# Mateng0228/Leak-det-gnn

Hardware: AMD Instinct MI355X
Metric: windowed graphs/sec fwd+bwd on L-TOWN-A (higher is better)
Workload: dtype fp32; 1 GPU; L-TOWN-A detector training step (BASELINE configs[2]); graph=L-TOWN-A, nodes=661, edge_columns=1532, pipes=764, windows_per_rank=256, global_batch=256, feat=64, gnn_layers=2, parallelism=dp1, launch=hipgraph (one replay per step, dropout re-drawn on device)

## Files before the change

include/leakgnn.h:

```cpp
#ifndef LEAKGNN_H
#define LEAKGNN_H

#include <stdint.h>

#ifdef __cplusplus
extern "C" {
#endif

typedef void* lg_stream_t;

enum {
    LG_OK = 0,
    LG_EINVAL = -1,
    LG_EUNSUPPORTED = -2,
    LG_EHIP = -3
};

#define LG_F_BIAS      0x01
#define LG_F_RELU      0x02
#define LG_F_DROPOUT   0x04
#define LG_F_MASK_IN   0x08
#define LG_F_MASK_OUT  0x10
#define LG_F_DX_SENSOR_ROWS 0x10000000
#define LG_F_NODE_MAJOR 0x20
#define LG_F_BF16 0x40
#define LG_SALT_SEED_PTR 0x80000000u
#define LG_F_F32_MFMA      0x00400000
#define LG_F_PC            0x00004000
#define LG_F_BF16X3        0x00008000
#define LG_F_NM3           0x00020000

int lg_abi_version(void);

int lg_reduce_batch_begin(void);
int lg_reduce_batch_flush(lg_stream_t stream);

int lg_stream_copy(const void* src, void* dst, int64_t bytes, lg_stream_t stream);

int lg_seed_slots_advance(uint64_t* slots, int64_t n, uint64_t* state, lg_stream_t stream);

int lg_graph_replay(void* graph_exec, int64_t n, lg_stream_t stream);
const char* lg_strerror(int code);

int lg_cross_entropy_fwd(const float* logits, const int64_t* target, int64_t B, int64_t C, int64_t ldx,
                         int64_t ignore_index, float* loss, float* lse, float* rowloss, unsigned* counter,
                         lg_stream_t stream);
int lg_cross_entropy_bwd(const float* logits, const int64_t* target, const float* lse, const float* grad_loss,
                         int64_t B, int64_t C, int64_t ldx, int64_t ignore_index, float* dlogits, int64_t ldd,
                         lg_stream_t stream);

int64_t lg_clip_adamw_workspace_bytes(const int64_t* sizes, int T);
int lg_clip_adamw(const int64_t* table, const int64_t* sizes, int T, float* step, float lr, float beta1,
                  float beta2, float eps, float weight_decay, float max_norm, float* norm_out, void* workspace, int64_t ws_bytes,
                  lg_stream_t stream);
int lg_clip_adamw_seeds(const int64_t* table, const int64_t* sizes, int T, float* step, float lr, float beta1,
                        float beta2, float eps, float weight_decay, float max_norm, float* norm_out, void* workspace,
                        int64_t ws_bytes, uint64_t* seed_slots, int64_t n_slots, uint64_t* seed_state,
                        lg_stream_t stream);

int lg_spin_errors(uint32_t* out, int reset);

int lg_timing_arm(int slot);
int lg_timing_disarm(void);
int lg_timing_elapsed(int slot, float* ms);

int64_t lg_graph_workspace_bytes(int64_t E, int64_t N);
int lg_graph_build(const int64_t* edge_index, int64_t E, int64_t N,
                   int add_self_loops, int normalize, float fill_value,
                   int32_t* rowptr, int32_t* col, float* w,
                   int32_t* rowptr_t, int32_t* col_t, float* w_t,
                   void* workspace, int64_t ws_bytes, lg_stream_t stream);

int64_t lg_graph_build_w_workspace_bytes(int64_t E, int64_t N);
int lg_graph_build_w(const int64_t* edge_index, const float* edge_weight, int64_t E, int64_t N,
                     int add_self_loops, int normalize, float fill_value,
                     int32_t* rowptr, int32_t* col, float* w, int32_t* eid,
                     int32_t* rowptr_t, int32_t* col_t, float* w_t, int32_t* eid_t, float* dis,
                     void* workspace, int64_t ws_bytes, lg_stream_t stream);
int lg_graph_reweight(const int32_t* rowptr, const int32_t* col, const int32_t* eid,
                      const int32_t* rowptr_t, const int32_t* col_t, const int32_t* eid_t,
                      const float* edge_weight, int64_t E, int64_t N, int normalize, float fill_value,
                      float* dis, float* w, float* w_t, lg_stream_t stream);
int64_t lg_gcn_norm_bwd_workspace_bytes(int64_t E, int64_t N);
int lg_gcn_norm_bwd(const float* G, const int32_t* rowptr, const int32_t* col, const int32_t* eid,
                    const int32_t* rowptr_t, const int32_t* col_t, const int32_t* eid_t,
                    const float* dis, const float* edge_weight, int64_t E, int64_t N, int normalize,
                    float fill_value, float* dedge_weight, void* workspace, int64_t ws_bytes,
                    lg_stream_t stream);

int lg_sddmm_cols(const int32_t* rowptr, const int32_t* col, const float* a, int64_t lda,
                  const float* b, int64_t ldb, float* out, int64_t N, int64_t C, lg_stream_t stream);

int lg_nm_table_build(const int32_t* rowptr, const int32_t* pairs, int64_t N, const int32_t* order,
                      int32_t* nodetab, lg_stream_t stream);

int lg_nm_table_sensor_mark(const int32_t* nodetab, const int32_t* pairs, int64_t N, int64_t nnz,
                            const int32_t* node_slot, int32_t* nodetab_out, int32_t* pairs_out, int32_t* pos_slot,
                            lg_stream_t stream);

int lg_rcm_order(const int64_t* edge_index, int64_t E, int64_t N, int32_t* order);

int64_t lg_incidence_workspace_bytes(int64_t P, int64_t N);
int lg_incidence_build(const int64_t* ends, int64_t P, int64_t N,
                       int32_t* inc_rowptr, int32_t* inc_item,
                       void* workspace, int64_t ws_bytes, lg_stream_t stream);

int lg_batchify_edge_index(const int64_t* edge_index, int64_t E, int64_t N, int64_t B,
                           int64_t* out, lg_stream_t stream);

int lg_node_init_fwd(const int32_t* sensor_slot, const float* proj, const float* bias, float* x0,
                     int64_t B, int64_t N, int64_t S, int64_t D,
                     int flags, float dropout_p, uint64_t seed, uint32_t salt, lg_stream_t stream);

int lg_node_init_proj_fwd(const int32_t* sensor_slot, const int64_t* sensor_idx, const float* h_s, const float* W,
                          const float* bias, float* x0, int64_t B, int64_t N, int64_t S, int64_t Ds, int64_t D,
                          int flags, float dropout_p, uint64_t seed, uint32_t salt, lg_stream_t stream);

int64_t lg_sensor_proj_bwd_workspace_bytes(int64_t B, int64_t S, int64_t Ds, int64_t D);
int lg_sensor_proj_bwd(const float* dx0, const int64_t* sensor_idx, const float* live, const float* h_s,
                       const float* W, const float* dbias_in, float* dh_s, float* dW, float* db, int64_t B,
                       int64_t N, int64_t S, int64_t Ds, int64_t D, int flags, void* workspace, int64_t ws_bytes,
                       lg_stream_t stream);

int64_t lg_linear_dw_workspace_bytes(int64_t K, int64_t M, int64_t N);
int lg_linear_dw(const float* dy, const float* x, int64_t K, int64_t M, int64_t N,
                 float* dw, float* db, void* workspace, int64_t ws_bytes, lg_stream_t stream);

int lg_gcn_fwd(const int32_t* rowptr, const int32_t* col, const float* w,
               const float* x, const float* W, const float* bias, float* y,
               int64_t B, int64_t N, int64_t D, int64_t nnz_cap,
               int flags, float dropout_p, uint64_t seed, uint32_t salt, lg_stream_t stream);

// ... 178 lines not shown
```

leak-det-gnn_amd/csrc/loss.hip:

```cpp
#include <algorithm>
#include "common.h"

namespace {

constexpr int kCeWaves = 4;
constexpr int kCeThreads = 64 * kCeWaves;
constexpr int kCePer = 16;
constexpr float kCeLseFine = 32.f;

__device__ __forceinline__ float wave_max(float v) {
#pragma unroll
    for (int o = 32; o > 0; o >>= 1) v = fmaxf(v, __shfl_xor(v, o));
    return v;
}
__device__ __forceinline__ float wave_sum(float v) {
#pragma unroll
    for (int o = 32; o > 0; o >>= 1) v += __shfl_xor(v, o);
    return v;
}

__device__ __forceinline__ void ce_mean_wave(float* rowloss, const int64_t* __restrict__ target, int64_t B,
                                             int64_t ignore, float* __restrict__ loss) {
    const int lane = threadIdx.x & 63;
    float acc = 0.f, cnt = 0.f;
    for (int64_t b0 = 0; b0 < B; b0 += 64) {
        const int64_t b = b0 + lane;
        float v = 0.f, c = 0.f;
        if (b < B) {
            v = __hip_atomic_load(rowloss + b, __ATOMIC_RELAXED, __HIP_MEMORY_SCOPE_AGENT);
            c = target[b] == ignore ? 0.f : 1.f;
        }
        acc += wave_sum(v);
        cnt += wave_sum(c);
    }
    if (lane == 0) loss[0] = acc / cnt;
}

__global__ void __launch_bounds__(kCeThreads)
k_ce_fwd(const float* __restrict__ x, const int64_t* __restrict__ target, int64_t B, int64_t C, int64_t ldx,
         int64_t ignore, float* __restrict__ lse, float* rowloss, unsigned* counter, float* __restrict__ loss) {
    __shared__ unsigned is_last;
    const int w = threadIdx.x >> 6, lane = threadIdx.x & 63;
    for (int64_t b = static_cast<int64_t>(blockIdx.x) * kCeWaves + w; b < B; b += static_cast<int64_t>(gridDim.x) * kCeWaves) {
        const float* row = x + b * ldx;
        float m = -__builtin_huge_valf(), s = 0.f;
        if (C <= 64 * kCePer) {
            float v[kCePer];
#pragma unroll
            for (int k = 0; k < kCePer; ++k) {
                const int64_t c = lane + 64 * k;
                v[k] = c < C ? row[c] : -__builtin_huge_valf();
            }
#pragma unroll
            for (int k = 0; k < kCePer; ++k) m = fmaxf(m, v[k]);
            m = wave_max(m);
#pragma unroll
            for (int k = 0; k < kCePer; ++k) s += lane + 64 * k < C ? expf(v[k] - m) : 0.f;
        } else {
            for (int64_t c = lane; c < C; c += 64) m = fmaxf(m, row[c]);
            m = wave_max(m);
            for (int64_t c = lane; c < C; c += 64) s += expf(row[c] - m);
        }
        s = wave_sum(s);
        const float ls = logf(s);
        const float l = m + ls;
        if (lane == 0) {
            const int64_t t = target[b];
            lse[b] = l;
            float rl = t == ignore ? 0.f : __builtin_nanf("");
            if (t >= 0 && t < C && t != ignore) rl = fabsf(l) < kCeLseFine ? l - row[t] : (m - row[t]) + ls;
            __hip_atomic_store(rowloss + b, rl, __ATOMIC_RELAXED, __HIP_MEMORY_SCOPE_AGENT);
        }
    }
    asm volatile("s_waitcnt vmcnt(0)" ::: "memory");
    __syncthreads();
    if (threadIdx.x == 0) {
        const unsigned old = __hip_atomic_fetch_add(counter, 1u, __ATOMIC_RELAXED, __HIP_MEMORY_SCOPE_AGENT);
        is_last = old + 1 == gridDim.x ? 1u : 0u;
    }
    __syncthreads();
    if (!is_last) return;
    if (w == 0) ce_mean_wave(rowloss, target, B, ignore, loss);
    if (threadIdx.x == 0) __hip_atomic_store(counter, 0u, __ATOMIC_RELAXED, __HIP_MEMORY_SCOPE_AGENT);
}

__global__ void __launch_bounds__(kCeThreads)
k_ce_bwd(const float* __restrict__ x, const int64_t* __restrict__ target, const float* __restrict__ lse,
         const float* __restrict__ gout, int64_t B, int64_t C, int64_t ldx, int64_t ignore, float* __restrict__ dx,
         int64_t ldd) {
    const int w = threadIdx.x >> 6, lane = threadIdx.x & 63;
    float cnt = 0.f;
    for (int64_t b0 = 0; b0 < B; b0 += 64) {
        const int64_t b = b0 + lane;
        cnt += wave_sum((b < B && target[b] != ignore) ? 1.f : 0.f);
    }
    const float g = gout[0] / cnt;
    for (int64_t b = static_cast<int64_t>(blockIdx.x) * kCeWaves + w; b < B; b += static_cast<int64_t>(gridDim.x) * kCeWaves) {
        const float* row = x + b * ldx;
        float* drow = dx + b * ldd;
        const int64_t t = target[b];
        const float l = lse[b];
        const float gi = t == ignore ? 0.f : g;
        const bool fine = fabsf(l) < kCeLseFine;
        if (C <= 64 * kCePer) {
            float v[kCePer];
#pragma unroll
            for (int k = 0; k < kCePer; ++k) {
                const int64_t c = lane + 64 * k;
                v[k] = c < C ? row[c] : 0.f;
            }
            if (fine) {
#pragma unroll
                for (int k = 0; k < kCePer; ++k) {
                    const int64_t c = lane + 64 * k;
                    if (c < C) drow[c] = gi * (expf(v[k] - l) - (c == t ? 1.f : 0.f));
                }
            } else {
                float m = -__builtin_huge_valf(), s = 0.f;
#pragma unroll
                for (int k = 0; k < kCePer; ++k) m = lane + 64 * k < C ? fmaxf(m, v[k]) : m;
                m = wave_max(m);
#pragma unroll
                for (int k = 0; k < kCePer; ++k) {
                    v[k] = lane + 64 * k < C ? expf(v[k] - m) : 0.f;
                    s += v[k];
                }
                const float rs = 1.f / wave_sum(s);
#pragma unroll
                for (int k = 0; k < kCePer; ++k) {
                    const int64_t c = lane + 64 * k;
                    if (c < C) drow[c] = gi * (v[k] * rs - (c == t ? 1.f : 0.f));
                }
            }
        } else if (fine) {
            for (int64_t c = lane; c < C; c += 64) drow[c] = gi * (expf(row[c] - l) - (c == t ? 1.f : 0.f));
        } else {
            float m = -__builtin_huge_valf(), s = 0.f;
            for (int64_t c = lane; c < C; c += 64) m = fmaxf(m, row[c]);
            m = wave_max(m);
            for (int64_t c = lane; c < C; c += 64) s += expf(row[c] - m);
            const float rs = 1.f / wave_sum(s);
            for (int64_t c = lane; c < C; c += 64) drow[c] = gi * (expf(row[c] - m) * rs - (c == t ? 1.f : 0.f));
        }
    }
}

}

extern "C" int lg_cross_entropy_fwd(const float* logits, const int64_t* target, int64_t B, int64_t C, int64_t ldx,
                                    int64_t ignore_index, float* loss, float* lse, float* rowloss, unsigned* counter,
                                    lg_stream_t stream) {
    if (B < 0 || C <= 0 || ldx < C || !loss || !counter) return LG_EINVAL;
    hipStream_t s = lg_stream(stream);
    if (B == 0) {
        return hipMemsetD32Async(reinterpret_cast<hipDeviceptr_t>(loss), 0x7FC00000, 1, s) == hipSuccess ? LG_OK
                                                                                                          : LG_EHIP;
    }
    if (!logits || !target || !lse || !rowloss) return LG_EINVAL;
    const int grid = static_cast<int>(std::min<int64_t>((B + kCeWaves - 1) / kCeWaves, lg_num_cus()));
    lg_launch(k_ce_fwd, grid, kCeThreads, 0, s, logits, target, B, C, ldx, ignore_index, lse, rowloss, counter, loss);
    LG_RET_IF_LAUNCH_FAILED();
    return LG_OK;
}

extern "C" int lg_cross_entropy_bwd(const float* logits, const int64_t* target, const float* lse,
                                    const float* grad_loss, int64_t B, int64_t C, int64_t ldx, int64_t ignore_index,
                                    float* dlogits, int64_t ldd, lg_stream_t stream) {
    if (B < 0 || C <= 0 || ldx < C || ldd < C || !grad_loss) return LG_EINVAL;
    if (B == 0) return LG_OK;
    if (!logits || !target || !lse || !dlogits) return LG_EINVAL;
    hipStream_t s = lg_stream(stream);
    const int grid = static_cast<int>(std::min<int64_t>((B + kCeWaves - 1) / kCeWaves, 4 * lg_num_cus()));
    lg_launch(k_ce_bwd, grid, kCeThreads, 0, s, logits, target, lse, grad_loss, B, C, ldx, ignore_index, dlogits, ldd);
    LG_RET_IF_LAUNCH_FAILED();
    return LG_OK;
}
```

leak-det-gnn_amd/csrc/optim.hip:

```cpp
#include <algorithm>
#include <cstdlib>
#include "common.h"

namespace {

constexpr int kOptThreads = 1024;
constexpr int kOptChunk = kOptThreads;
constexpr int kOptMaxTensors = 48;
constexpr uint32_t kOptPollLimit = 1u << 22;

struct AdamTensors {
    int64_t ptr[kOptMaxTensors][4];
    int64_t off[kOptMaxTensors + 1];
    int T;
};

__device__ __forceinline__ uint64_t opt_splitmix64(uint64_t z) {
    z += 0x9E3779B97F4A7C15ull;
    z = (z ^ (z >> 30)) * 0xBF58476D1CE4E5B9ull;
    z = (z ^ (z >> 27)) * 0x94D049BB133111EBull;
    return z ^ (z >> 31);
}
struct AdamSeeds {
    uint64_t* slots;
    uint64_t* state;
    int n;
};

enum : int {
    kAdamOne = 0,
    kAdamPartials = 1,
    kAdamNoNorm = 2,
};

__device__ __forceinline__ double opt_block_sum(double x, double* wsum) {
#pragma unroll
    for (int o = 32; o > 0; o >>= 1) x += __shfl_xor(x, o);
    if ((threadIdx.x & 63) == 0) wsum[threadIdx.x >> 6] = x;
    __syncthreads();
    double s = 0.0;
#pragma unroll
    for (int w = 0; w < kOptThreads / 64; ++w) s += wsum[w];
    __syncthreads();
    return s;
}

__device__ __forceinline__ int opt_tensor_of(const AdamTensors& a, int64_t e) {
    int t = 0;
    while (t < a.T && a.off[t + 1] <= e) ++t;
    return t;
}

__global__ void __launch_bounds__(kOptThreads) k_adam_partials(AdamTensors a, double* __restrict__ partials) {
    __shared__ double wsum[kOptThreads / 64];
    const int64_t e = static_cast<int64_t>(blockIdx.x) * kOptChunk + threadIdx.x;
    const int t = opt_tensor_of(a, e);
    double x = 0.0;
    if (t < a.T) x = reinterpret_cast<const float*>(a.ptr[t][1])[e - a.off[t]];
    const double s = opt_block_sum(x * x, wsum);
    if (threadIdx.x == 0) partials[blockIdx.x] = s;
}

template <int MODE>
__global__ void __launch_bounds__(kOptThreads)
k_adam(AdamTensors a, float* __restrict__ step, float lr, float beta1, float beta2, float eps, float wd,
       float max_norm, float* __restrict__ norm_out, double* __restrict__ partials, int skew, AdamSeeds seeds) {
    __shared__ uint32_t last;
    __shared__ double wsum[kOptThreads / 64];
    __shared__ float tsh;
    const int tid = threadIdx.x;
    const uint32_t G = gridDim.x;
    uint32_t* ctr = reinterpret_cast<uint32_t*>(step + 1);
    if (tid == 0) tsh = __hip_atomic_load(step, __ATOMIC_RELAXED, __HIP_MEMORY_SCOPE_AGENT) + 1.0f;
    if (MODE == kAdamNoNorm) __syncthreads();
    const int64_t e = static_cast<int64_t>(blockIdx.x) * kOptChunk + tid;
    const int t = opt_tensor_of(a, e);
    const bool live = t < a.T;
    const int64_t i = live ? e - a.off[t] : 0;
    float* p = live ? reinterpret_cast<float*>(a.ptr[t][0]) : nullptr;
    float* g = live ? reinterpret_cast<float*>(a.ptr[t][1]) : nullptr;
    float* m = live ? reinterpret_cast<float*>(a.ptr[t][2]) : nullptr;
    float* v = live ? reinterpret_cast<float*>(a.ptr[t][3]) : nullptr;
    if (MODE == kAdamOne && skew > 0 && (blockIdx.x & 1)) {
        for (int k = 0; k < skew; ++k) __builtin_amdgcn_s_sleep(127);
    }
    float gi = live ? g[i] : 0.0f;
    double norm = 0.0;
    if (MODE == kAdamOne) {
        const double s = opt_block_sum(static_cast<double>(gi) * gi, wsum);
        if (tid == 0) {
            partials[blockIdx.x] = s;
            __hip_atomic_fetch_add(ctr, 1u, __ATOMIC_RELEASE, __HIP_MEMORY_SCOPE_AGENT);
            uint32_t polls = 0;
            while (__hip_atomic_load(ctr, __ATOMIC_RELAXED, __HIP_MEMORY_SCOPE_AGENT) < G) {
                if (++polls > kOptPollLimit) {
                    __hip_atomic_fetch_or(reinterpret_cast<uint32_t*>(step + 2), 1u, __ATOMIC_RELAXED,
                                          __HIP_MEMORY_SCOPE_AGENT);
                    break;
                }
                __builtin_amdgcn_s_sleep(2);
            }
            __builtin_amdgcn_fence(__ATOMIC_ACQUIRE, "agent");
        }
        __syncthreads();
    }
    if (MODE != kAdamNoNorm) {
        double s = 0.0;
        for (uint32_t j = tid; j < G; j += kOptThreads) s += partials[j];
        norm = sqrt(opt_block_sum(s, wsum));
    }
    const float t1 = tsh;
    if (tid == 0) {
        if (MODE != kAdamOne)
            asm volatile("s_waitcnt vmcnt(0) lgkmcnt(0)" ::: "memory");
        const uint32_t tk = __hip_atomic_fetch_add(ctr, 1u, __ATOMIC_RELAXED, __HIP_MEMORY_SCOPE_AGENT);
        last = tk + 1 == (MODE == kAdamOne ? 2 * G : G) ? 1u : 0u;
        if (last) {
            __hip_atomic_store(step, t1, __ATOMIC_RELAXED, __HIP_MEMORY_SCOPE_AGENT);
            __hip_atomic_store(ctr, 0u, __ATOMIC_RELAXED, __HIP_MEMORY_SCOPE_AGENT);
        }
        if (blockIdx.x == 0 && norm_out) norm_out[0] = static_cast<float>(norm);
    }
    if (seeds.slots) {
        __syncthreads();
        if (last && tid < 64) {
            const uint64_t c = seeds.state[0] + 1;
            for (int k = tid; k < seeds.n; k += 64)
                seeds.slots[k] = opt_splitmix64(c * static_cast<uint64_t>(seeds.n) + static_cast<uint64_t>(k) + 1) &
                                 ((1ull << 62) - 1);
            if (tid == 0) seeds.state[0] = c;
        }
    }
    if (!live) return;
    const double ratio = static_cast<double>(max_norm) / (norm + 1e-6);
    const float coef = max_norm > 0.f ? static_cast<float>(ratio >= 1.0 ? 1.0 : ratio) : 1.0f;
    const float bc1 = 1.0f - powf(beta1, t1), bc2 = 1.0f - powf(beta2, t1);
    const float step_size = lr / bc1, bc2s = sqrtf(bc2), decay = 1.0f - lr * wd;
    if (max_norm > 0.f) {
        gi *= coef;
        g[i] = gi;
    }
    const float pi = p[i] * decay;
    const float mi = beta1 * m[i] + (1.0f - beta1) * gi;
    const float vi = beta2 * v[i] + (1.0f - beta2) * gi * gi;
    m[i] = mi;
    v[i] = vi;
    p[i] = pi - step_size * mi / (sqrtf(vi) / bc2s + eps);
}

}

extern "C" int64_t lg_clip_adamw_workspace_bytes(const int64_t* sizes, int T) {
    if (T < 0 || T > kOptMaxTensors || (T > 0 && !sizes)) return LG_EUNSUPPORTED;
    int64_t n = 0;
    for (int t = 0; t < T; ++t) n += std::max<int64_t>(sizes[t], 0);
    return 8 * std::max<int64_t>(1, (n + kOptChunk - 1) / kOptChunk);
}

namespace {
int env_int(const char* name) {
    const char* s = getenv(name);
    return s ? atoi(s) : 0;
}

int clip_adamw_impl(const int64_t* table, const int64_t* sizes, int T, float* step, float lr, float beta1, float beta2,
                    float eps, float weight_decay, float max_norm, float* norm_out, void* workspace, int64_t ws_bytes,
                    const AdamSeeds& seeds, lg_stream_t stream) {
    if (T > kOptMaxTensors) return LG_EUNSUPPORTED;
    if (T < 0 || (T > 0 && (!table || !sizes)) || !step || !workspace) return LG_EINVAL;
    if (!(beta1 >= 0.f && beta1 < 1.f) || !(beta2 >= 0.f && beta2 < 1.f) || !(eps >= 0.f)) return LG_EINVAL;
    AdamTensors a{};
    a.off[0] = 0;
    for (int t = 0; t < T; ++t) {
        for (int j = 0; j < 4; ++j) {
            if (!table[4 * t + j]) return LG_EINVAL;
            a.ptr[t][j] = table[4 * t + j];
        }
        if (sizes[t] < 0) return LG_EINVAL;
        a.off[t + 1] = a.off[t] + sizes[t];
    }
    a.T = T;
    const int64_t G64 = std::max<int64_t>(1, (a.off[T] + kOptChunk - 1) / kOptChunk);
    if (G64 > 0x3fffffff) return LG_EUNSUPPORTED;
    if (ws_bytes < 8 * G64) return LG_EINVAL;
    const int G = static_cast<int>(G64);
    double* partials = static_cast<double*>(workspace);
    hipStream_t s = lg_stream(stream);
    if (!(max_norm > 0.f) && !norm_out) {
        lg_launch(k_adam<kAdamNoNorm>, G, kOptThreads, 0, s, a, step, lr, beta1, beta2, eps, weight_decay, max_norm,
                  norm_out, partials, 0, seeds);
    } else if (G <= lg_num_cus() && !env_int("LEAKGNN_LAB_ADAM_TWO_LAUNCH")) {
        lg_launch(k_adam<kAdamOne>, G, kOptThreads, 0, s, a, step, lr, beta1, beta2, eps, weight_decay, max_norm,
                  norm_out, partials, env_int("LEAKGNN_LAB_ADAM_SKEW"), seeds);
    } else {
        hipLaunchKernelGGL(k_adam_partials, dim3(G), dim3(kOptThreads), 0, s, a, partials);
        LG_RET_IF_LAUNCH_FAILED();
        lg_launch(k_adam<kAdamPartials>, G, kOptThreads, 0, s, a, step, lr, beta1, beta2, eps, weight_decay,
                  max_norm, norm_out, partials, 0, seeds);
    }
    LG_RET_IF_LAUNCH_FAILED();
    return LG_OK;
}
}

extern "C" int lg_clip_adamw(const int64_t* table, const int64_t* sizes, int T, float* step, float lr, float beta1,
                             float beta2, float eps, float weight_decay, float max_norm, float* norm_out,
                             void* workspace, int64_t ws_bytes, lg_stream_t stream) {
    return clip_adamw_impl(table, sizes, T, step, lr, beta1, beta2, eps, weight_decay, max_norm, norm_out, workspace,
                           ws_bytes, AdamSeeds{nullptr, nullptr, 0}, stream);
}

extern "C" int lg_clip_adamw_seeds(const int64_t* table, const int64_t* sizes, int T, float* step, float lr,
                                   float beta1, float beta2, float eps, float weight_decay, float max_norm,
                                   float* norm_out, void* workspace, int64_t ws_bytes, uint64_t* seed_slots,
                                   int64_t n_slots, uint64_t* seed_state, lg_stream_t stream) {
    if (n_slots < 0 || n_slots > 4096 || (n_slots > 0 && (!seed_slots || !seed_state))) return LG_EINVAL;
    return clip_adamw_impl(table, sizes, T, step, lr, beta1, beta2, eps, weight_decay, max_norm, norm_out, workspace,
                           ws_bytes, AdamSeeds{n_slots > 0 ? seed_slots : nullptr, seed_state, static_cast<int>(n_slots)},
                           stream);
}
```

leak-det-gnn_amd/models/_native.py:

```python
from __future__ import annotations

import ctypes
import os
from pathlib import Path

import torch

_PKG_ROOT = Path(__file__).resolve().parent.parent
LIB_PATH = Path(os.environ.get("LEAKGNN_LIB", _PKG_ROOT / "lib" / "libleakgnn.so"))

ABI_VERSION = 26

LG_F_BIAS = 0x01
LG_F_RELU = 0x02
LG_F_DROPOUT = 0x04
LG_F_MASK_IN = 0x08
LG_F_MASK_OUT = 0x10
LG_F_NODE_MAJOR = 0x20
LG_F_DX_SENSOR_ROWS = 0x10000000
LG_SALT_SEED_PTR = 0x80000000
LG_F_F32_MFMA = 0x00400000
LG_F_BF16 = 0x40
LG_F_PC = 0x00004000
LG_F_BF16X3 = 0x00008000
LG_F_NM3 = 0x00020000

_i32, _i64, _u32, _u64, _f32, _p = (ctypes.c_int, ctypes.c_int64, ctypes.c_uint32, ctypes.c_uint64,
                                    ctypes.c_float, ctypes.c_void_p)

SIGNATURES = {
    "lg_abi_version": (_i32, []),
    "lg_strerror": (ctypes.c_char_p, [_i32]),
    "lg_reduce_batch_begin": (_i32, []),
    "lg_reduce_batch_flush": (_i32, [_p]),
    "lg_stream_copy": (_i32, [_p, _p, _i64, _p]),
    "lg_seed_slots_advance": (_i32, [_p, _i64, _p, _p]),
    "lg_graph_replay": (_i32, [_p, _i64, _p]),
    "lg_cross_entropy_fwd": (_i32, [_p, _p, _i64, _i64, _i64, _i64, _p, _p, _p, _p, _p]),
    "lg_cross_entropy_bwd": (_i32, [_p, _p, _p, _p, _i64, _i64, _i64, _i64, _p, _i64, _p]),
    "lg_clip_adamw_workspace_bytes": (_i64, [_p, _i32]),
    "lg_clip_adamw": (_i32, [_p, _p, _i32, _p, _f32, _f32, _f32, _f32, _f32, _f32, _p, _p, _i64, _p]),
    "lg_clip_adamw_seeds": (_i32, [_p, _p, _i32, _p, _f32, _f32, _f32, _f32, _f32, _f32, _p, _p, _i64, _p, _i64, _p,
                                   _p]),
    "lg_spin_errors": (_i32, [_p, _i32]),
    "lg_timing_arm": (_i32, [_i32]),
    "lg_timing_disarm": (_i32, []),
    "lg_timing_elapsed": (_i32, [_i32, _p]),
    "lg_graph_workspace_bytes": (_i64, [_i64, _i64]),
    "lg_graph_build": (_i32, [_p, _i64, _i64, _i32, _i32, _f32, _p, _p, _p, _p, _p, _p, _p, _i64, _p]),
    "lg_graph_build_w_workspace_bytes": (_i64, [_i64, _i64]),
    "lg_graph_build_w": (_i32, [_p, _p, _i64, _i64, _i32, _i32, _f32, _p, _p, _p, _p, _p, _p, _p, _p, _p, _p, _i64, _p]),
    "lg_graph_reweight": (_i32, [_p, _p, _p, _p, _p, _p, _p, _i64, _i64, _i32, _f32, _p, _p, _p, _p]),
    "lg_gcn_norm_bwd_workspace_bytes": (_i64, [_i64, _i64]),
    "lg_gcn_norm_bwd": (_i32, [_p, _p, _p, _p, _p, _p, _p, _p, _p, _i64, _i64, _i32, _f32, _p, _p, _i64, _p]),
    "lg_sddmm_cols": (_i32, [_p, _p, _p, _i64, _p, _i64, _p, _i64, _i64, _p]),
    "lg_nm_table_build": (_i32, [_p, _p, _i64, _p, _p, _p]),
    "lg_rcm_order": (_i32, [_p, _i64, _i64, _p]),
    "lg_incidence_workspace_bytes": (_i64, [_i64, _i64]),
    "lg_incidence_build": (_i32, [_p, _i64, _i64, _p, _p, _p, _i64, _p]),
    "lg_batchify_edge_index": (_i32, [_p, _i64, _i64, _i64, _p, _p]),
    "lg_linear_dw_workspace_bytes": (_i64, [_i64, _i64, _i64]),
    "lg_linear_dw": (_i32, [_p, _p, _i64, _i64, _i64, _p, _p, _p, _i64, _p]),
    "lg_node_init_fwd": (_i32, [_p, _p, _p, _p, _i64, _i64, _i64, _i64, _i32, _f32, _u64, _u32, _p]),
    "lg_node_init_proj_fwd": (_i32, [_p, _p, _p, _p, _p, _p, _i64, _i64, _i64, _i64, _i64, _i32, _f32, _u64, _u32,
                                     _p]),
    "lg_sensor_proj_bwd_workspace_bytes": (_i64, [_i64, _i64, _i64, _i64]),
    "lg_sensor_proj_bwd": (_i32, [_p, _p, _p, _p, _p, _p, _p, _p, _p, _i64, _i64, _i64, _i64, _i64, _i32, _p, _i64, _p]),
    "lg_gcn_fwd": (_i32, [_p, _p, _p, _p, _p, _p, _p, _i64, _i64, _i64, _i64, _i32, _f32, _u64, _u32, _p]),
    "lg_spmm": (_i32, [_p, _p, _p, _p, _p, _i64, _i64, _i64, _i64, _p]),
    "lg_spmm_cols": (_i32, [_p, _p, _p, _p, _i64, _p, _p, _i64, _i64, _i64, _p]),
    "lg_gcn_bwd_workspace_bytes": (_i64, [_i64]),
    "lg_gcn_bwd": (_i32, [_p, _p, _p, _p, _p, _p, _p, _p, _p, _p, _p, _p, _i64, _i64, _i64, _i64, _i32, _f32, _f32, _p, _i64, _p]),
    "lg_pipe_gather_fwd": (_i32, [_p, _p, _p, _i64, _i64, _i64, _i64, _p]),
    "lg_pipe_scatter_bwd": (_i32, [_p, _p, _p, _p, _p, _i64, _i64, _i64, _i64, _i32, _p]),
    "lg_gcn_fwd_nm": (_i32, [_p, _p, _p, _p, _p, _p, _i64, _i64, _i64, _i64, _i32, _f32, _u64, _u32, _p]),
    "lg_gcn_fwd_nm_bits": (_i32, [_p, _p, _p, _p, _p, _p, _i64, _i64, _i64, _i64, _i32, _f32, _u64, _u32, _p, _p]),
    "lg_nm_table_sensor_mark": (_i32, [_p, _p, _i64, _i64, _p, _p, _p, _p, _p]),
    "lg_node_init_bits_fwd": (_i32, [_p, _p, _p, _p, _p, _p, _p, _i64, _i64, _i64, _i64, _i64, _i32, _f32, _u64, _u32,
                                     _p]),
    "lg_node_init_expand": (_i32, [_p, _p, _p, _p, _p, _i64, _i64, _i64, _i32, _f32, _p]),
    "lg_gcn_fwd_nm_x0": (_i32, [_p, _p, _p, _p, _p, _p, _p, _p, _i64, _i64, _i64, _i64, _i32, _f32, _u64, _u32, _p]),
    "lg_gcn_bwd_nm_x0": (_i32, [_p, _p, _p, _p, _p, _p, _p, _p, _p, _p, _p, _p, _p, _i64, _i64, _i64, _i64, _i32,
                                _f32, _f32, _p, _i64, _p]),
    "lg_gcn_fwd_rows": (_i32, [_p, _p, _p, _p, _p, _p, _i64, _i64, _i32, _p]),
    "lg_gcn_bwd_rows": (_i32, [_p, _p, _p, _p, _p, _p, _p, _p, _i64, _i64, _p, _i64, _p]),
    "lg_gcn_bwd_nm_bits": (_i32, [_p, _p, _p, _p, _p, _p, _p, _p, _p, _p, _p, _i64, _i64, _i64, _i32, _f32, _f32, _p, _i64, _p, _p]),
    "lg_gcn_bwd_nm_workspace_bytes": (_i64, [_i64]),
    "lg_gcn_bwd_nm": (_i32, [_p, _p, _p, _p, _p, _p, _p, _p, _p, _p, _p, _i64, _i64, _i64, _i32, _f32, _f32, _p, _i64, _p]),
    "lg_edge_head_fwd": (_i32, [_p, _p, _p, _p, _p, _p, _p, _i64, _p, _i64, _i64, _i64, _i64, _i64, _i32, _f32,
                                _u64, _u32, _p]),
    "lg_edge_head_bwd_workspace_bytes": (_i64, [_i64, _i64, _i64, _i64]),
    "lg_edge_head_bwd": (_i32, [_p, _p, _p, _p, _p, _p, _i64, _p, _p, _p, _p, _p, _i64, _i64, _i64, _i64, _i64, _i32, _f32, _p, _i64, _p]),
    "lg_edge_head_bwd_scatter": (_i32, [_p, _p, _p, _p, _p, _p, _i64, _p, _p, _p, _p, _p, _p, _p, _p, _p, _p, _p, _i64, _i64,
                                        _i64, _i64, _i64, _i32, _f32, _p, _i64, _p]),
    "lg_pipe_schedule_words": (_i64, [_i64, _i64, _i64]),
    "lg_pipe_schedule_build": (_i32, [_p, _i64, _i64, _i64, _p, _i64, _p, _p]),
    "lg_mean_pool_fwd": (_i32, [_p, _p, _i64, _i64, _i64, _p]),
    "lg_pool_head_fwd": (_i32, [_p, _p, _p, _p, _p, _p, _p, _p, _i64, _i64, _i64, _i64, _i64, _i64, _i32, _f32, _u64,
                                _u32, _p]),
    "lg_pool_head_bwd_workspace_bytes": (_i64, [_i64, _i64, _i64]),
    "lg_pool_head_bwd": (_i32, [_p, _p, _p, _p, _p, _i64, _i64, _p, _p, _p, _p, _p, _i64, _i64, _i64, _i32, _f32, _p, _i64, _p]),
    "lg_heads_bwd_scatter": (_i32, [_p, _p, _p, _p, _p, _p, _p, _p, _i32, _f32, _p, _i64,
                                    _p, _p, _p, _p, _p, _p, _i64, _p, _p, _p, _p, _p, _p, _p, _p, _p, _p, _p,
                                    _i64, _i64, _i64, _i64, _i64, _i32, _f32, _p, _i64, _p]),
    "lg_gru_fwd": (_i32, [_p, _p, _p, _p, _p, _p, _p, _p, _p, _i64, _i64, _i64, _i64, _i64, _p]),
    "lg_gru_bwd_workspace_bytes": (_i64, [_i64, _i64, _i64, _i64]),
    "lg_gru_bwd": (_i32, [_p, _p, _p, _p, _p, _p, _p, _p, _p, _p, _p, _p, _i64, _i64, _i64, _i64, _i64, _p, _i64, _p]),
    "lg_gru_seq_fwd": (_i32, [_p, _p, _p, _p, _p, _p, _p, _i64, _i64, _i64, _i64, _i32, _f32, _u64, _u32, _p]),
    "lg_gru_seq_bwd_workspace_bytes": (_i64, [_i64, _i64, _i64]),
    "lg_gru_seq_tiled": (_i32, [_i64, _i64, _i32]),
    "lg_gru_seq_infer": (_i32, [_p, _p, _p, _p, _p, _p, _p, _i64, _i64, _i64, _i64, _i32, _f32, _u64, _u32, _p]),
    "lg_gru_win_fwd": (_i32, [_p, _p, _p, _p, _p, _i64, _i64, _i64, _i64, _i64, _p]),
    "lg_gru_seq_bwd": (_i32, [_p, _p, _p, _p, _p, _p, _p, _p, _p, _p, _p, _p, _p, _p, _i64, _i64, _i64, _i64, _i64,
                              _i64, _i32, _f32, _u64, _u32, _p, _i64, _p]),
    "lg_gru_node_init_fwd": (_i32, [_p, _p, _p, _p, _p, _p, _p, _p, _p, _p, _p, _p, _p, _p, _p,
                                    _i64, _i64, _i64, _i64, _i64, _i64, _i32, _f32, _u64, _u32, _p]),
    "lg_gru_node_init_bwd_workspace_bytes": (_i64, [_i64, _i64, _i64, _i64]),
    "lg_gru_node_init_bwd": (_i32, [_p, _p, _p, _p, _p, _p, _p, _p, _p, _p, _p, _p, _p, _p, _p, _p, _p,
                                    _i64, _i64, _i64, _i64, _i64, _i64, _p, _i64, _p]),
    "lg_tcn_packed_weight_floats": (_i64, [_i64]),
    "lg_tcn_pack_weight": (_i32, [_p, _p, _i64, _p]),
    "lg_tcn_conv_fwd": (_i32, [_p, _p, _p, _p, _p, _p, _p, _f32, _p, _i64, _i64, _i64, _i64, _i64, _p]),
# ... 59 lines not shown
```

leak-det-gnn_amd/models/graph_step.py:

```python
from __future__ import annotations

from typing import Callable, Optional, Sequence

import torch
import torch.distributed as dist

from . import ops


def _world() -> int:
    return dist.get_world_size() if (dist.is_available() and dist.is_initialized()) else 1


class CapturedTrainStep:

    def __init__(self, model: torch.nn.Module, loss_fn: Callable, opt: torch.optim.Optimizer,
                 inputs: Sequence[torch.Tensor], label: torch.Tensor, clip: Optional[float] = 1.0,
                 warmup: int = 3, seed_slots: int = 16, preserve_state: bool = False):
        for group in opt.param_groups:
            if not group.get("capturable", False):
                raise ValueError("CapturedTrainStep needs an optimizer built with capturable=True")
        self.model, self.loss_fn, self.opt, self.clip = model, loss_fn, opt, clip
        self.inputs, self.label = tuple(inputs), label
        self.params = [p for p in model.parameters() if p.requires_grad]
        dev = label.device
        self.world = _world()
        self.slots = ops.SeedSlots(dev, seed_slots)
        self._one: Optional[torch.Tensor] = None
        self._build(model, warmup, preserve_state)

    def _build(self, model, warmup: int, preserve_state: bool) -> None:
        dev = self.label.device
        snap = self._snapshot() if preserve_state else None
        side = torch.cuda.Stream(dev)
        side.wait_stream(torch.cuda.current_stream(dev))
        with torch.cuda.stream(side):
            for _ in range(warmup):
                self._eager_step()
        torch.cuda.current_stream(dev).wait_stream(side)
        torch.cuda.synchronize(dev)

        self.opt.zero_grad(set_to_none=True)
        self.comm = True
        self.graph_a = torch.cuda.CUDAGraph()
        self.graph_a2 = None
        self.graph_b = None
        split = getattr(model, "overlap_split", None)
        self.heads = [p for p in split() if p.requires_grad] if (self.world > 1 and split is not None) else []
        hid = {id(p) for p in self.heads}
        self.trunk = [p for p in self.params if id(p) not in hid]
        ops.use_device_seeds(self.slots)
        self.fold_seeds = hasattr(self.opt, "seed_slots")
        head_refresh = not self.fold_seeds
        try:
            if self.world == 1:
                with torch.cuda.graph(self.graph_a):
                    if head_refresh:
                        self.slots.refresh()
                    self.loss = self._forward_backward().detach()
                    self._update(fold=self.fold_seeds)
            elif self.heads:
                model.keep_boundary = True
                try:
                    with torch.cuda.graph(self.graph_a):
                        if head_refresh:
                            self.slots.refresh()
                        loss = self.loss_fn(self.model(*self.inputs), self.label)
                        bnd = model.boundary
                        self._one = torch.ones_like(loss)
                        torch.autograd.backward(loss, self._one, retain_graph=True, inputs=self.heads + [bnd])
                        self.loss = loss.detach()
                        self.flat_h = torch.cat([p.grad.reshape(-1) for p in self.heads])
                    self.graph_a2 = torch.cuda.CUDAGraph()
                    with torch.cuda.graph(self.graph_a2, pool=self.graph_a.pool()):
                        torch.autograd.backward(bnd, bnd.grad, inputs=self.trunk)
                        self.flat_t = torch.cat([p.grad.reshape(-1) for p in self.trunk])
                finally:
                    model.keep_boundary = False
                    model.boundary = None
                del loss, bnd
                self.buckets = [(self.flat_h, self.heads), (self.flat_t, self.trunk)]
            else:
                with torch.cuda.graph(self.graph_a):
                    if head_refresh:
                        self.slots.refresh()
                    self.loss = self._forward_backward().detach()
                    self.flat = torch.cat([p.grad.reshape(-1) for p in self.params])
                self.buckets = [(self.flat, self.params)]
        finally:
            ops.use_device_seeds(None)
        if snap is not None:
            self._restore(snap)
        if self.fold_seeds and self.world == 1:
            self.slots.refresh()
            torch.cuda.synchronize(dev)
        if self.world > 1:
            grads, views = [], []
            for flat, ps in self.buckets:
                off = 0
                for p in ps:
                    grads.append(p.grad)
                    views.append(flat[off:off + p.numel()].view_as(p))
                    off += p.numel()
            self.graph_b = torch.cuda.CUDAGraph()
            with torch.cuda.graph(self.graph_b):
                torch._foreach_copy_(grads, views)
                self._update(fold=self.fold_seeds)
            if self.fold_seeds:
                self.slots.refresh()
                torch.cuda.synchronize(dev)

    def _opt_tensors(self) -> list:
        out = []
        for st in self.opt.state.values():
            out += [v for v in st.values() if torch.is_tensor(v)]
        for g in self.opt.param_groups:
            out += [v for v in g.values() if torch.is_tensor(v)]
        return out

    def _snapshot(self) -> tuple:
        with torch.no_grad():
            params = [(p, p.detach().clone()) for p in self.model.parameters()]
            opt = {id(t): (t, t.detach().clone()) for t in self._opt_tensors()}
        return params, opt, torch.get_rng_state()

    def _restore(self, snap: tuple) -> None:
        params, opt, rng = snap
        with torch.no_grad():
            for p, v in params:
                p.copy_(v)
            for t in self._opt_tensors():
                if id(t) in opt:
                    t.copy_(opt[id(t)][1])
                else:
                    t.zero_()
        torch.set_rng_state(rng)
        torch.cuda.synchronize()

    def _forward_backward(self) -> torch.Tensor:
        loss = self.loss_fn(self.model(*self.inputs), self.label)
        if self._one is None or self._one.shape != loss.shape:
            self._one = torch.ones_like(loss)
        loss.backward(self._one)
        return loss

    def _update(self, fold: bool = False) -> None:
        if self.clip is not None:
            torch.nn.utils.clip_grad_norm_(self.params, self.clip)
        if fold:
            self.opt.seed_slots = self.slots
        try:
            self.opt.step()
        finally:
            if fold:
                self.opt.seed_slots = None

    def _eager_step(self) -> None:
        self.opt.zero_grad(set_to_none=True)
        self._forward_backward()
        if self.world > 1:
            flat = torch.cat([p.grad.reshape(-1) for p in self.params])
            dist.all_reduce(flat, op=dist.ReduceOp.SUM)
            flat.div_(self.world)
            off = 0
            for p in self.params:
                p.grad.copy_(flat[off:off + p.numel()].view_as(p))
                off += p.numel()
        self._update()

    def _all_reduce(self, flat: torch.Tensor, async_op: bool = False):
        if dist.get_backend() == "nccl":
            return dist.all_reduce(flat, op=dist.ReduceOp.AVG, async_op=async_op)
        work = dist.all_reduce(flat, op=dist.ReduceOp.SUM, async_op=async_op)
        if work is not None:
            work.wait()
        flat.div_(self.world)
        return None

    def __call__(self) -> torch.Tensor:
        self.graph_a.replay()
        if self.graph_b is not None:
            if self.graph_a2 is not None:
                work = self._all_reduce(self.flat_h, async_op=True) if self.comm else None
                self.graph_a2.replay()
                if self.comm:
                    self._all_reduce(self.flat_t)
                    if work is not None:
                        work.wait()
            elif self.comm:
                self._all_reduce(self.flat)
            self.graph_b.replay()
        return self.loss
```

leak-det-gnn_amd/models/loss.py:

```python
from __future__ import annotations

from typing import Tuple

import torch
from torch import Tensor

from ._native import check, load_library, ptr, stream_of

NS = "leakgnn"
_POOL_SLOTS = 256
_POOLS: dict = {}
_SLOTS: dict = {}


def _counter(dev: torch.device, stream: int) -> Tensor:
    key = (dev, stream)
    i = _SLOTS.get(key)
    pool = _POOLS.get(dev)
    if pool is None:
        if torch.cuda.is_current_stream_capturing():
            raise RuntimeError("leakgnn cross_entropy: run the loss once eagerly before capturing it "
                               "(its counter pool is allocated on the first call)")
        pool = _POOLS[dev] = torch.zeros(_POOL_SLOTS, dtype=torch.int32, device=dev)
    if i is None:
        i = len([k for k in _SLOTS if k[0] == dev])
        if i >= _POOL_SLOTS:
            raise RuntimeError(f"leakgnn cross_entropy: more than {_POOL_SLOTS} streams on {dev}")
        _SLOTS[key] = i
    return pool[i:i + 1]


@torch.library.custom_op(f"{NS}::cross_entropy", mutates_args=(), device_types="cuda")
def cross_entropy(logits: Tensor, target: Tensor, ignore_index: int) -> Tuple[Tensor, Tensor]:
    lib = load_library()
    x, t = logits.contiguous(), target.contiguous()
    B, C = x.shape
    loss = torch.empty((), device=x.device, dtype=torch.float32)
    lse = torch.empty(B, device=x.device, dtype=torch.float32)
    rowloss = torch.empty(B, device=x.device, dtype=torch.float32)
    st = stream_of(x)
    check(lib.lg_cross_entropy_fwd(ptr(x), ptr(t), B, C, C, ignore_index, ptr(loss), ptr(lse), ptr(rowloss),
                                   ptr(_counter(x.device, st)), st), "lg_cross_entropy_fwd")
    return loss, lse


@cross_entropy.register_fake
def _(logits, target, ignore_index):
    return logits.new_empty(()), logits.new_empty(logits.shape[0])


@torch.library.custom_op(f"{NS}::cross_entropy_backward", mutates_args=(), device_types="cuda")
def cross_entropy_backward(grad: Tensor, logits: Tensor, target: Tensor, lse: Tensor, ignore_index: int) -> Tensor:
    lib = load_library()
    x, t, g = logits.contiguous(), target.contiguous(), grad.contiguous().float()
    B, C = x.shape
    dx = torch.empty_like(x)
    check(lib.lg_cross_entropy_bwd(ptr(x), ptr(t), ptr(lse), ptr(g), B, C, C, ignore_index, ptr(dx), C,
                                   stream_of(x)), "lg_cross_entropy_bwd")
    return dx


@cross_entropy_backward.register_fake
def _(grad, logits, target, lse, ignore_index):
    return torch.empty_like(logits)


def _ce_setup(ctx, inputs, output):
    logits, target, ignore_index = inputs
    ctx.ignore_index = ignore_index
    ctx.mark_non_differentiable(output[1])
    ctx.set_materialize_grads(False)
    ctx.save_for_backward(logits, target, output[1])


def _ce_bwd(ctx, g, _glse):
    if g is None:
        return None, None, None
    logits, target, lse = ctx.saved_tensors
    return torch.ops.leakgnn.cross_entropy_backward(g, logits, target, lse, ctx.ignore_index), None, None


cross_entropy.register_autograd(_ce_bwd, setup_context=_ce_setup)


class CrossEntropyLoss(torch.nn.CrossEntropyLoss):

    def forward(self, input: Tensor, target: Tensor) -> Tensor:
        if (self.weight is None and self.reduction == "mean" and self.label_smoothing == 0.0 and input.is_cuda
                and input.dim() == 2 and input.dtype == torch.float32 and target.dtype == torch.int64
                and target.dim() == 1):
            return torch.ops.leakgnn.cross_entropy(input, target, int(self.ignore_index))[0]
        return super().forward(input, target)
```

Baseline: 502,400 windows/s.

## Fuse cross-entropy gradient into forward kernel when upstream grad is unit

Adds a fused forward+grad cross-entropy kernel that writes dlogits during the forward pass from the logits already held in registers. Autograd returns that precomputed gradient when the seed gradient is the known unit tensor, which removes the separate backward kernel launch and its re-read of the logits. The Adam single-launch path also switches to relaxed atomics with an explicit waitcnt instead of release/acquire fences, and reserves 96KB of dynamic LDS, apparently to limit each CU to one resident block. The cost is an extra forward-time write and the fused path's reliance on pointer identity of the unit seed.

```diff
diff --git a/include/leakgnn.h b/include/leakgnn.h
--- a/include/leakgnn.h
+++ b/include/leakgnn.h
@@ -48,6 +48,9 @@
 int lg_cross_entropy_bwd(const float* logits, const int64_t* target, const float* lse, const float* grad_loss,
                          int64_t B, int64_t C, int64_t ldx, int64_t ignore_index, float* dlogits, int64_t ldd,
                          lg_stream_t stream);
+int lg_cross_entropy_fwd_grad(const float* logits, const int64_t* target, int64_t B, int64_t C, int64_t ldx,
+                              int64_t ignore_index, float* loss, float* lse, float* rowloss, unsigned* counter,
+                              float* du, int64_t ldd, lg_stream_t stream);
 
 int64_t lg_clip_adamw_workspace_bytes(const int64_t* sizes, int T);
 int lg_clip_adamw(const int64_t* table, const int64_t* sizes, int T, float* step, float lr, float beta1,
diff --git a/leak-det-gnn_amd/csrc/loss.hip b/leak-det-gnn_amd/csrc/loss.hip
--- a/leak-det-gnn_amd/csrc/loss.hip
+++ b/leak-det-gnn_amd/csrc/loss.hip
@@ -36,16 +36,71 @@
     if (lane == 0) loss[0] = acc / cnt;
 }
 
+__device__ __forceinline__ float ce_count_rows(const int64_t* __restrict__ target, int64_t B, int64_t ignore) {
+    const int lane = threadIdx.x & 63;
+    float cnt = 0.f;
+    for (int64_t b0 = 0; b0 < B; b0 += 64) {
+        const int64_t b = b0 + lane;
+        cnt += wave_sum((b < B && target[b] != ignore) ? 1.f : 0.f);
+    }
+    return cnt;
+}
+
+__device__ __forceinline__ void ce_row_grad_regs(float (&v)[kCePer], float* __restrict__ drow, int64_t C, int64_t t,
+                                                 float l, float gi, int lane) {
+    if (fabsf(l) < kCeLseFine) {
+#pragma unroll
+        for (int k = 0; k < kCePer; ++k) {
+            const int64_t c = lane + 64 * k;
+            if (c < C) drow[c] = gi * (expf(v[k] - l) - (c == t ? 1.f : 0.f));
+        }
+    } else {
+        float m = -__builtin_huge_valf(), s = 0.f;
+#pragma unroll
+        for (int k = 0; k < kCePer; ++k) m = lane + 64 * k < C ? fmaxf(m, v[k]) : m;
+        m = wave_max(m);
+#pragma unroll
+        for (int k = 0; k < kCePer; ++k) {
+            v[k] = lane + 64 * k < C ? expf(v[k] - m) : 0.f;
+            s += v[k];
+        }
+        const float rs = 1.f / wave_sum(s);
+#pragma unroll
+        for (int k = 0; k < kCePer; ++k) {
+            const int64_t c = lane + 64 * k;
+            if (c < C) drow[c] = gi * (v[k] * rs - (c == t ? 1.f : 0.f));
+        }
+    }
+}
+
+__device__ __forceinline__ void ce_row_grad_loop(const float* __restrict__ row, float* __restrict__ drow, int64_t C,
+                                                 int64_t t, float l, float gi, int lane) {
+    if (fabsf(l) < kCeLseFine) {
+        for (int64_t c = lane; c < C; c += 64) drow[c] = gi * (expf(row[c] - l) - (c == t ? 1.f : 0.f));
+    } else {
+        float m = -__builtin_huge_valf(), s = 0.f;
+        for (int64_t c = lane; c < C; c += 64) m = fmaxf(m, row[c]);
+        m = wave_max(m);
+        for (int64_t c = lane; c < C; c += 64) s += expf(row[c] - m);
+        const float rs = 1.f / wave_sum(s);
+        for (int64_t c = lane; c < C; c += 64) drow[c] = gi * (expf(row[c] - m) * rs - (c == t ? 1.f : 0.f));
+    }
+}
+
+template <bool GRAD>
 __global__ void __launch_bounds__(kCeThreads)
 k_ce_fwd(const float* __restrict__ x, const int64_t* __restrict__ target, int64_t B, int64_t C, int64_t ldx,
-         int64_t ignore, float* __restrict__ lse, float* rowloss, unsigned* counter, float* __restrict__ loss) {
+         int64_t ignore, float* __restrict__ lse, float* rowloss, unsigned* counter, float* __restrict__ loss,
+         float* __restrict__ du, int64_t ldd) {
     __shared__ unsigned is_last;
     const int w = threadIdx.x >> 6, lane = threadIdx.x & 63;
+    float g = 0.f;
+    if (GRAD) g = 1.0f / ce_count_rows(target, B, ignore);
     for (int64_t b = static_cast<int64_t>(blockIdx.x) * kCeWaves + w; b < B; b += static_cast<int64_t>(gridDim.x) * kCeWaves) {
         const float* row = x + b * ldx;
         float m = -__builtin_huge_valf(), s = 0.f;
+        float v[kCePer];
         if (C <= 64 * kCePer) {
-            float v[kCePer];
 #pragma unroll
             for (int k = 0; k < kCePer; ++k) {
                 const int64_t c = lane + 64 * k;
@@ -71,6 +126,14 @@
             if (t >= 0 && t < C && t != ignore) rl = fabsf(l) < kCeLseFine ? l - row[t] : (m - row[t]) + ls;
             __hip_atomic_store(rowloss + b, rl, __ATOMIC_RELAXED, __HIP_MEMORY_SCOPE_AGENT);
         }
+        if (GRAD) {
+            const int64_t t = target[b];
+            const float gi = t == ignore ? 0.f : g;
+            if (C <= 64 * kCePer)
+                ce_row_grad_regs(v, du + b * ldd, C, t, l, gi, lane);
+            else
+                ce_row_grad_loop(row, du + b * ldd, C, t, l, gi, lane);
+        }
     }
     asm volatile("s_waitcnt vmcnt(0)" ::: "memory");
     __syncthreads();
@@ -89,19 +152,13 @@
          const float* __restrict__ gout, int64_t B, int64_t C, int64_t ldx, int64_t ignore, float* __restrict__ dx,
          int64_t ldd) {
     const int w = threadIdx.x >> 6, lane = threadIdx.x & 63;
-    float cnt = 0.f;
-    for (int64_t b0 = 0; b0 < B; b0 += 64) {
-        const int64_t b = b0 + lane;
-        cnt += wave_sum((b < B && target[b] != ignore) ? 1.f : 0.f);
-    }
-    const float g = gout[0] / cnt;
+    const float g = gout[0] / ce_count_rows(target, B, ignore);
     for (int64_t b = static_cast<int64_t>(blockIdx.x) * kCeWaves + w; b < B; b += static_cast<int64_t>(gridDim.x) * kCeWaves) {
         const float* row = x + b * ldx;
         float* drow = dx + b * ldd;
         const int64_t t = target[b];
         const float l = lse[b];
         const float gi = t == ignore ? 0.f : g;
-        const bool fine = fabsf(l) < kCeLseFine;
         if (C <= 64 * kCePer) {
             float v[kCePer];
 #pragma unroll
@@ -109,47 +166,19 @@
                 const int64_t c = lane + 64 * k;
                 v[k] = c < C ? row[c] : 0.f;
             }
-            if (fine) {
-#pragma unroll
-                for (int k = 0; k < kCePer; ++k) {
-                    const int64_t c = lane + 64 * k;
-                    if (c < C) drow[c] = gi * (expf(v[k] - l) - (c == t ? 1.f : 0.f));
-                }
-            } else {
-                float m = -__builtin_huge_valf(), s = 0.f;
-#pragma unroll
-                for (int k = 0; k < kCePer; ++k) m = lane + 64 * k < C ? fmaxf(m, v[k]) : m;
-                m = wave_max(m);
-#pragma unroll
-                for (int k = 0; k < kCePer; ++k) {
-                    v[k] = lane + 64 * k < C ? expf(v[k] - m) : 0.f;
-                    s += v[k];
-                }
-                const float rs = 1.f / wave_sum(s);
-#pragma unroll
-                for (int k = 0; k < kCePer; ++k) {
-                    const int64_t c = lane + 64 * k;
-                    if (c < C) drow[c] = gi * (v[k] * rs - (c == t ? 1.f : 0.f));
-                }
-            }
-        } else if (fine) {
-            for (int64_t c = lane; c < C; c += 64) drow[c] = gi * (expf(row[c] - l) - (c == t ? 1.f : 0.f));
+            ce_row_grad_regs(v, drow, C, t, l, gi, lane);
         } else {
-            float m = -__builtin_huge_valf(), s = 0.f;
-            for (int64_t c = lane; c < C; c += 64) m = fmaxf(m, row[c]);
-            m = wave_max(m);
-            for (int64_t c = lane; c < C; c += 64) s += expf(row[c] - m);
-            const float rs = 1.f / wave_sum(s);
-            for (int64_t c = lane; c < C; c += 64) drow[c] = gi * (expf(row[c] - m) * rs - (c == t ? 1.f : 0.f));
-        }
-    }
-}
-
-}
-
-extern "C" int lg_cross_entropy_fwd(const float* logits, const int64_t* target, int64_t B, int64_t C, int64_t ldx,
-                                    int64_t ignore_index, float* loss, float* lse, float* rowloss, unsigned* counter,
-                                    lg_stream_t stream) {
+            ce_row_grad_loop(row, drow, C, t, l, gi, lane);
+        }
+    }
+}
+
+}
+
+namespace {
+int ce_fwd_impl(const float* logits, const int64_t* target, int64_t B, int64_t C, int64_t ldx, int64_t ignore_index,
+                float* loss, float* lse, float* rowloss, unsigned* counter, float* du, int64_t ldd,
+                lg_stream_t stream) {
     if (B < 0 || C <= 0 || ldx < C || !loss || !counter) return LG_EINVAL;
     hipStream_t s = lg_stream(stream);
     if (B == 0) {
@@ -157,10 +186,30 @@
                                                                                                           : LG_EHIP;
     }
     if (!logits || !target || !lse || !rowloss) return LG_EINVAL;
+    if (du && (ldd < C || du == logits)) return LG_EINVAL;
     const int grid = static_cast<int>(std::min<int64_t>((B + kCeWaves - 1) / kCeWaves, lg_num_cus()));
-    lg_launch(k_ce_fwd, grid, kCeThreads, 0, s, logits, target, B, C, ldx, ignore_index, lse, rowloss, counter, loss);
+    if (du)
+        lg_launch(k_ce_fwd<true>, grid, kCeThreads, 0, s, logits, target, B, C, ldx, ignore_index, lse, rowloss,
+                  counter, loss, du, ldd);
+    else
+        lg_launch(k_ce_fwd<false>, grid, kCeThreads, 0, s, logits, target, B, C, ldx, ignore_index, lse, rowloss,
+                  counter, loss, du, ldd);
     LG_RET_IF_LAUNCH_FAILED();
     return LG_OK;
+}
+}
+
+extern "C" int lg_cross_entropy_fwd(const float* logits, const int64_t* target, int64_t B, int64_t C, int64_t ldx,
+                                    int64_t ignore_index, float* loss, float* lse, float* rowloss, unsigned* counter,
+                                    lg_stream_t stream) {
+    return ce_fwd_impl(logits, target, B, C, ldx, ignore_index, loss, lse, rowloss, counter, nullptr, 0, stream);
+}
+
+extern "C" int lg_cross_entropy_fwd_grad(const float* logits, const int64_t* target, int64_t B, int64_t C, int64_t ldx,
+                                         int64_t ignore_index, float* loss, float* lse, float* rowloss,
+                                         unsigned* counter, float* du, int64_t ldd, lg_stream_t stream) {
+    if (B > 0 && !du) return LG_EINVAL;
+    return ce_fwd_impl(logits, target, B, C, ldx, ignore_index, loss, lse, rowloss, counter, du, ldd, stream);
 }
 
 extern "C" int lg_cross_entropy_bwd(const float* logits, const int64_t* target, const float* lse,
diff --git a/leak-det-gnn_amd/csrc/optim.hip b/leak-det-gnn_amd/csrc/optim.hip
--- a/leak-det-gnn_amd/csrc/optim.hip
+++ b/leak-det-gnn_amd/csrc/optim.hip
@@ -8,6 +8,7 @@
 constexpr int kOptChunk = kOptThreads;
 constexpr int kOptMaxTensors = 48;
 constexpr uint32_t kOptPollLimit = 1u << 22;
+constexpr int kAdamOneLds = 96 * 1024;
 
 struct AdamTensors {
     int64_t ptr[kOptMaxTensors][4];
@@ -64,7 +65,7 @@
 template <int MODE>
 __global__ void __launch_bounds__(kOptThreads)
 k_adam(AdamTensors a, float* __restrict__ step, float lr, float beta1, float beta2, float eps, float wd,
-       float max_norm, float* __restrict__ norm_out, double* __restrict__ partials, int skew, AdamSeeds seeds) {
+       float max_norm, float* __restrict__ norm_out, double* partials, int skew, AdamSeeds seeds) {
     __shared__ uint32_t last;
     __shared__ double wsum[kOptThreads / 64];
     __shared__ float tsh;
@@ -89,8 +90,9 @@
     if (MODE == kAdamOne) {
         const double s = opt_block_sum(static_cast<double>(gi) * gi, wsum);
         if (tid == 0) {
-            partials[blockIdx.x] = s;
-            __hip_atomic_fetch_add(ctr, 1u, __ATOMIC_RELEASE, __HIP_MEMORY_SCOPE_AGENT);
+            __hip_atomic_store(partials + blockIdx.x, s, __ATOMIC_RELAXED, __HIP_MEMORY_SCOPE_AGENT);
+            asm volatile("s_waitcnt vmcnt(0)" ::: "memory");
+            __hip_atomic_fetch_add(ctr, 1u, __ATOMIC_RELAXED, __HIP_MEMORY_SCOPE_AGENT);
             uint32_t polls = 0;
             while (__hip_atomic_load(ctr, __ATOMIC_RELAXED, __HIP_MEMORY_SCOPE_AGENT) < G) {
                 if (++polls > kOptPollLimit) {
@@ -100,13 +102,14 @@
                 }
                 __builtin_amdgcn_s_sleep(2);
             }
-            __builtin_amdgcn_fence(__ATOMIC_ACQUIRE, "agent");
         }
         __syncthreads();
     }
     if (MODE != kAdamNoNorm) {
         double s = 0.0;
-        for (uint32_t j = tid; j < G; j += kOptThreads) s += partials[j];
+        for (uint32_t j = tid; j < G; j += kOptThreads)
+            s += MODE == kAdamOne ? __hip_atomic_load(partials + j, __ATOMIC_RELAXED, __HIP_MEMORY_SCOPE_AGENT)
+                                  : partials[j];
         norm = sqrt(opt_block_sum(s, wsum));
     }
     const float t1 = tsh;
@@ -190,7 +193,10 @@
         lg_launch(k_adam<kAdamNoNorm>, G, kOptThreads, 0, s, a, step, lr, beta1, beta2, eps, weight_decay, max_norm,
                   norm_out, partials, 0, seeds);
     } else if (G <= lg_num_cus() && !env_int("LEAKGNN_LAB_ADAM_TWO_LAUNCH")) {
-        lg_launch(k_adam<kAdamOne>, G, kOptThreads, 0, s, a, step, lr, beta1, beta2, eps, weight_decay, max_norm,
+        if (hipFuncSetAttribute(reinterpret_cast<const void*>(k_adam<kAdamOne>),
+                                hipFuncAttributeMaxDynamicSharedMemorySize, kAdamOneLds) != hipSuccess)
+            return LG_EHIP;
+        lg_launch(k_adam<kAdamOne>, G, kOptThreads, kAdamOneLds, s, a, step, lr, beta1, beta2, eps, weight_decay, max_norm,
                   norm_out, partials, env_int("LEAKGNN_LAB_ADAM_SKEW"), seeds);
     } else {
         hipLaunchKernelGGL(k_adam_partials, dim3(G), dim3(kOptThreads), 0, s, a, partials);
diff --git a/leak-det-gnn_amd/models/_native.py b/leak-det-gnn_amd/models/_native.py
--- a/leak-det-gnn_amd/models/_native.py
+++ b/leak-det-gnn_amd/models/_native.py
@@ -38,6 +38,7 @@
     "lg_graph_replay": (_i32, [_p, _i64, _p]),
     "lg_cross_entropy_fwd": (_i32, [_p, _p, _i64, _i64, _i64, _i64, _p, _p, _p, _p, _p]),
     "lg_cross_entropy_bwd": (_i32, [_p, _p, _p, _p, _i64, _i64, _i64, _i64, _p, _i64, _p]),
+    "lg_cross_entropy_fwd_grad": (_i32, [_p, _p, _i64, _i64, _i64, _i64, _p, _p, _p, _p, _p, _i64, _p]),
     "lg_clip_adamw_workspace_bytes": (_i64, [_p, _i32]),
     "lg_clip_adamw": (_i32, [_p, _p, _i32, _p, _f32, _f32, _f32, _f32, _f32, _f32, _p, _p, _i64, _p]),
     "lg_clip_adamw_seeds": (_i32, [_p, _p, _i32, _p, _f32, _f32, _f32, _f32, _f32, _f32, _p, _p, _i64, _p, _i64, _p,
diff --git a/leak-det-gnn_amd/models/graph_step.py b/leak-det-gnn_amd/models/graph_step.py
--- a/leak-det-gnn_amd/models/graph_step.py
+++ b/leak-det-gnn_amd/models/graph_step.py
@@ -5,6 +5,7 @@
 import torch
 import torch.distributed as dist
 
+from . import loss as loss_mod
 from . import ops
 
 
@@ -67,7 +68,7 @@
                             self.slots.refresh()
                         loss = self.loss_fn(self.model(*self.inputs), self.label)
                         bnd = model.boundary
-                        self._one = torch.ones_like(loss)
+                        self._one = self._seed(loss)
                         torch.autograd.backward(loss, self._one, retain_graph=True, inputs=self.heads + [bnd])
                         self.loss = loss.detach()
                         self.flat_h = torch.cat([p.grad.reshape(-1) for p in self.heads])
@@ -137,10 +138,16 @@
         torch.set_rng_state(rng)
         torch.cuda.synchronize()
 
+    def _seed(self, loss: torch.Tensor) -> torch.Tensor:
+        if loss.dim() == 0 and loss.dtype == torch.float32 and loss.is_cuda:
+            return loss_mod.unit_grad(loss.device)
+        if self._one is None or self._one.shape != loss.shape or self._one.dtype != loss.dtype:
+            return torch.ones_like(loss)
+        return self._one
+
     def _forward_backward(self) -> torch.Tensor:
         loss = self.loss_fn(self.model(*self.inputs), self.label)
-        if self._one is None or self._one.shape != loss.shape:
-            self._one = torch.ones_like(loss)
+        self._one = self._seed(loss)
         loss.backward(self._one)
         return loss
 
diff --git a/leak-det-gnn_amd/models/loss.py b/leak-det-gnn_amd/models/loss.py
--- a/leak-det-gnn_amd/models/loss.py
+++ b/leak-det-gnn_amd/models/loss.py
@@ -11,6 +11,25 @@
 _POOL_SLOTS = 256
 _POOLS: dict = {}
 _SLOTS: dict = {}
+_UNIT: dict = {}
+
+
+def unit_grad(device) -> Tensor:
+    dev = torch.device(device)
+    if dev.type == "cuda" and dev.index is None:
+        dev = torch.device("cuda", torch.cuda.current_device())
+    one = _UNIT.get(dev)
+    if one is None:
+        if dev.type == "cuda" and torch.cuda.is_current_stream_capturing():
+            raise RuntimeError("leakgnn unit_grad: take it once before capturing (it is allocated on the first call)")
+        one = _UNIT[dev] = torch.ones((), device=dev, dtype=torch.float32)
+    return one
+
+
+def _is_unit(g: Tensor) -> bool:
+    one = _UNIT.get(g.device)
+    return (one is not None and g.dim() == 0 and g.dtype == torch.float32
+            and g.data_ptr() == one.data_ptr())
 
 
 def _counter(dev: torch.device, stream: int) -> Tensor:
@@ -49,6 +68,26 @@
     return logits.new_empty(()), logits.new_empty(logits.shape[0])
 
 
+@torch.library.custom_op(f"{NS}::cross_entropy_grad", mutates_args=(), device_types="cuda")
+def cross_entropy_grad(logits: Tensor, target: Tensor, ignore_index: int) -> Tuple[Tensor, Tensor, Tensor]:
+    lib = load_library()
+    x, t = logits.contiguous(), target.contiguous()
+    B, C = x.shape
+    loss = torch.empty((), device=x.device, dtype=torch.float32)
+    lse = torch.empty(B, device=x.device, dtype=torch.float32)
+    rowloss = torch.empty(B, device=x.device, dtype=torch.float32)
+    du = torch.empty_like(x)
+    st = stream_of(x)
+    check(lib.lg_cross_entropy_fwd_grad(ptr(x), ptr(t), B, C, C, ignore_index, ptr(loss), ptr(lse), ptr(rowloss),
+                                        ptr(_counter(x.device, st)), ptr(du), C, st), "lg_cross_entropy_fwd_grad")
+    return loss, lse, du
+
+
+@cross_entropy_grad.register_fake
+def _(logits, target, ignore_index):
+    return logits.new_empty(()), logits.new_empty(logits.shape[0]), torch.empty_like(logits)
+
+
 @torch.library.custom_op(f"{NS}::cross_entropy_backward", mutates_args=(), device_types="cuda")
 def cross_entropy_backward(grad: Tensor, logits: Tensor, target: Tensor, lse: Tensor, ignore_index: int) -> Tensor:
     lib = load_library()
@@ -83,11 +122,33 @@
 cross_entropy.register_autograd(_ce_bwd, setup_context=_ce_setup)
 
 
+def _ceg_setup(ctx, inputs, output):
+    logits, target, ignore_index = inputs
+    ctx.ignore_index = ignore_index
+    ctx.mark_non_differentiable(output[1], output[2])
+    ctx.set_materialize_grads(False)
+    ctx.save_for_backward(logits, target, output[1], output[2])
+
+
+def _ceg_bwd(ctx, g, _glse, _gdu):
+    if g is None:
+        return None, None, None
+    logits, target, lse, du = ctx.saved_tensors
+    if _is_unit(g):
+        return du, None, None
+    return torch.ops.leakgnn.cross_entropy_backward(g, logits, target, lse, ctx.ignore_index), None, None
+
+
+cross_entropy_grad.register_autograd(_ceg_bwd, setup_context=_ceg_setup)
+
+
 class CrossEntropyLoss(torch.nn.CrossEntropyLoss):
 
     def forward(self, input: Tensor, target: Tensor) -> Tensor:
         if (self.weight is None and self.reduction == "mean" and self.label_smoothing == 0.0 and input.is_cuda
                 and input.dim() == 2 and input.dtype == torch.float32 and target.dtype == torch.int64
                 and target.dim() == 1):
+            if input.requires_grad and torch.is_grad_enabled():
+                return torch.ops.leakgnn.cross_entropy_grad(input, target, int(self.ignore_index))[0]
             return torch.ops.leakgnn.cross_entropy(input, target, int(self.ignore_index))[0]
         return super().forward(input, target)
```

Result: no change. 507,400 windows/s (median of 6 runs) (+1.0%).
